# xiezheng-cs/PyTorch_Distributed_Template

Hardware: AMD Instinct MI355X
Metric: images/sec (node) ResNet-18 DDP bs=1200/GPU at 1/2/4/8 MI355X (higher is better)
Workload: dtype bf16; 1 GPU; model=resnet18, global_batch=1200, parallelism=dp1, per_gpu_batch=1200, sync_bn=False, engine=native-hip, comm=none, grad_compress=none

## Files before the change

csrc/bindings.cpp:

```cpp
#include <torch/extension.h>
#include <ATen/hip/HIPContext.h>
#include <c10/hip/HIPCachingAllocator.h>
#include <c10/hip/HIPGuard.h>

#include <cstdio>
#include <algorithm>
#include <map>
#include <memory>
#include <mutex>
#include <optional>
#include <vector>
#include <stdexcept>
#include <string>

#include "common.h"
#include "dtypes.h"
#include "kernels/bn.h"
#include "kernels/bnact.h"
#include "kernels/conv1x1.h"
#include "kernels/conv_fwd.h"
#include "kernels/conv_l1.h"
#include "kernels/conv_wgrad.h"
#include "kernels/dwconv.h"
#include "kernels/fp32.h"
// ... 130 lines not shown
    TORCH_CHECK(Pm > 0 && Qm > 0 && f[6] + C * f[2] * f[3] * K + (nslice - 1) * w_slice_stride <= w_numel, op,
                ": bad phase");
    a.pooff_h[i] = (int)f[0]; a.pooff_w[i] = (int)f[1]; a.pT[i] = (int)f[2]; a.pU[i] = (int)f[3];
    a.pioff_h[i] = (int)f[4]; a.pioff_w[i] = (int)f[5]; a.pwoff[i] = f[6];
    a.pPm[i] = (int)Pm; a.pQm[i] = (int)Qm;
    maxM = std::max(maxM, N * Pm * Qm);
  }
  TORCH_CHECK(maxM < (int64_t(1) << 31), op, ": N*Pm*Qm must be < 2^31 (32-bit pixel indexing)");
  a.M = maxM;
}

void conv_fwd(const Tensor& x, const Tensor& w, Tensor& y, const OptT& res, const OptT& stats, int64_t N, int64_t H,
              int64_t W, int64_t C, int64_t Kout, int64_t T, int64_t U, int64_t Pm, int64_t Qm, int64_t ist_h,
              int64_t ist_w, int64_t ioff_h, int64_t ioff_w, int64_t tstep_h, int64_t tstep_w, int64_t OH, int64_t OW,
              int64_t ost_h, int64_t ost_w, int64_t ooff_h, int64_t ooff_w, int64_t bm, int64_t bn, int64_t bk,
              int64_t cs) {
  const int dt = dt16(x, "x");
  if (cs <= 0) cs = C;
  TORCH_CHECK(dt16(w, "w") == dt && dt16(y, "y") == dt, "conv_fwd: mixed dtypes");
  TORCH_CHECK(x.numel() == N * H * W * cs, "conv_fwd: x has ", x.numel(), " elements, geometry needs ", N * H * W * cs);
  TORCH_CHECK(x.numel() < (int64_t(1) << 30) && w.numel() < (int64_t(1) << 30),
              "conv_fwd: operands exceed 2 GiB (32-bit buffer offsets)");
  int pair_skip = 0;
  if (cs != C) {
    const int rows = C == 64 ? 2 : 1;
    TORCH_CHECK(cs == 4 && (C == 32 || (C == 64 && bk == 64 && U == 1)) && tstep_w >= 0 && U >= 1 && ioff_h >= 0 &&
                    ioff_w >= 0 && (Pm - 1) * ist_h + ioff_h + (T - 1) * tstep_h + rows - 1 < H &&
                    ((Qm - 1) * ist_w + ioff_w + (U - 1) * tstep_w) * cs + 32 <= W * cs,
                "conv_fwd: window-mode geometry leaves the padded image");
    if (C == 64) pair_skip = (int)(W * cs - 32);
  }
  TORCH_CHECK(w.numel() == Kout * T * U * C, "conv_fwd: w size mismatch");
// ... 8 lines not shown
  if (res.has_value()) {
    TORCH_CHECK(res->numel() == y.numel(), "conv_fwd: residual size mismatch");
    a.res = p16(*res, "res");
  }
  const int64_t M = N * Pm * Qm;
  if (stats.has_value()) {
    TORCH_CHECK(stats->numel() >= pdt::kStatSlots * Kout * 2, "conv_fwd: stats buffer too small");
    a.stats = pd(*stats, "stats");
  }
  a.N = N; a.H = H; a.W = W; a.C = C; a.Kout = Kout; a.T = T; a.U = U; a.Pm = Pm; a.Qm = Qm; a.cs = cs;
  a.pair_skip = pair_skip;
  a.ist_h = ist_h; a.ist_w = ist_w; a.ioff_h = ioff_h; a.ioff_w = ioff_w; a.tstep_h = tstep_h; a.tstep_w = tstep_w;
  a.OH = OH; a.OW = OW; a.ost_h = ost_h; a.ost_w = ost_w; a.ooff_h = ooff_h; a.ooff_w = ooff_w;
  TORCH_CHECK(M < (int64_t(1) << 31), "conv_fwd: N*Pm*Qm must be < 2^31 (32-bit pixel indexing)");
  a.M = M;
  pdt::conv_fwd_launch(a, dt, (int)bm, (int)bn, (int)bk, cur_stream());
  launched("conv_fwd_launch");
}

bool conv_fwd_pre_supported(int64_t N, int64_t H, int64_t W) {
  pdt::ConvFwdArgs a{};
  set_fwd_geom(a, N, H, W, 64, 64, 3, 3, H, W, 1, 1);
  a.cs = 64;
  int flip = 0;
  return pdt::conv_l1_eligible(a, &flip);
}

void conv_fwd_pre(const Tensor& z, const Tensor& w, Tensor& y, const Tensor& stats, const Tensor& pre_coef, int64_t N,
                  int64_t H, int64_t W) {
  const int dt = dt16(z, "z");
// ... 49 lines not shown
                              int64_t Q, int64_t res_phase) {
  if (!(bnb == 2 || bnb == 3) || res_phase >= 0 || stride != 1 || phases.size() != 1 || H != P || W != Q) return 0;
  const auto& f = phases[0];
  if (f.size() < 6 || f[0] != 0 || f[1] != 0 || f[2] != 1 || f[3] != 1 || f[4] != 0 || f[5] != 0) return 0;
  const bool x_ok = pdt::conv1x1x_bnb_supported((int)K, (int)C);
  if ((K == 64 || (K == 128 && bnb == 2)) && C == 256 && pdt::conv1x1_c64_supported(64, C) &&
      !(pdt::conv1x1x_prefer_l1() && x_ok))
    return 1;
  return x_ok ? 2 : 0;
}

void conv_dgrad_impl(const Tensor& dy, const Tensor& wt, Tensor& dx, const OptT& res, int64_t N, int64_t P,
                     int64_t Q, int64_t K, int64_t C, int64_t H, int64_t W, int64_t stride,
                     const std::vector<std::vector<int64_t>>& phases, int64_t bm, int64_t bn, int64_t bk, int64_t bnb,
                     const OptT& bn_y1, const OptT& bn_coef1, const OptT& bn_y2, const OptT& bn_coef2,
                     const OptT& bn_mask, const OptT& bn_slots, int64_t res_phase) {
  const int dt = dt16(dy, "dy");
  TORCH_CHECK(dt16(wt, "wt") == dt && dt16(dx, "dx") == dt, "conv_dgrad: mixed dtypes");
  TORCH_CHECK(dy.numel() == N * P * Q * K && dx.numel() == N * H * W * C, "conv_dgrad: size mismatch");
  TORCH_CHECK(dy.numel() < (int64_t(1) << 30) && wt.numel() < (int64_t(1) << 30),
              "conv_dgrad: operands exceed 2 GiB (32-bit buffer offsets)");
  TORCH_CHECK(K % bk == 0 && C % bn == 0, "conv_dgrad: K % bk / C % bn must be 0");
  pdt::ConvFwdArgs a{};
  a.x = p16(dy, "dy");
  a.w = p16(wt, "wt");
  a.y = p16(dx, "dx");
  set_dgrad_geom("conv_dgrad", a, N, P, Q, K, C, H, W, stride, phases, wt.numel(), 1, 0);
  a.cs = K;
  TORCH_CHECK(res_phase < (int64_t)phases.size() && (res_phase < 0 || res.has_value()), "conv_dgrad: bad res_phase");
  if (res.has_value()) {
    if (res_phase >= 0) {
      const int64_t Pm = a.pPm[res_phase], Qm = a.pQm[res_phase];
// ... 31 lines not shown
  const int64_t pk = dgrad_persistent_kind(K, C, bnb, stride, phases, H, W, P, Q, res_phase);
  if (pk == 1) {
    pdt::conv1x1_c64_bnb_launch(a.x, a.w + a.pwoff[0], a.y, a.res, a.bn_y1, a.bn_coef1, bnb == 3 ? a.bn_y2 : nullptr,
                                bnb == 3 ? a.bn_coef2 : nullptr, a.bn_mask, a.stats, N * P * Q, (int)K, dt,
                                cur_stream());
    launched("conv1x1_c64_bnb");
    return;
  }
  if (pk == 2) {
    pdt::conv1x1x_bnb_launch(a.x, a.w + a.pwoff[0], a.y, a.res, a.bn_y1, a.bn_coef1, bnb == 3 ? a.bn_y2 : nullptr,
                             bnb == 3 ? a.bn_coef2 : nullptr, a.bn_mask, a.stats, N * P * Q, (int)K, (int)C, dt,
                             cur_stream());
    launched("conv1x1x_bnb");
    return;
  }
  pdt::conv_fwd_launch(a, dt, (int)bm, (int)bn, (int)bk, cur_stream());
  launched("conv_fwd_launch");
}

void conv_dgrad(const Tensor& dy, const Tensor& wt, Tensor& dx, const OptT& res, int64_t N, int64_t P, int64_t Q,
                int64_t K, int64_t C, int64_t H, int64_t W, int64_t stride, const std::vector<std::vector<int64_t>>& phases,
                int64_t bm, int64_t bn, int64_t bk) {
  conv_dgrad_impl(dy, wt, dx, res, N, P, Q, K, C, H, W, stride, phases, bm, bn, bk, 0, {}, {}, {}, {}, {}, {}, -1);
}

bool conv1x1_c64_supported(int64_t C, int64_t Kout) { return pdt::conv1x1_c64_supported((int)C, (int)Kout); }

void conv1x1_c64(const Tensor& x, const Tensor& w, Tensor& y, const OptT& stats, int64_t M, const OptT& pre) {
  const int dt = dt16(x, "x");
  TORCH_CHECK(dt16(w, "w") == dt && dt16(y, "y") == dt, "conv1x1_c64: mixed dtypes");
  TORCH_CHECK(x.numel() >= M * 64 && w.numel() == 256 * 64 && y.numel() >= M * 256, "conv1x1_c64: size mismatch");
  TORCH_CHECK(M * 256 < (int64_t(1) << 31), "conv1x1_c64: M*256 must be < 2^31 (32-bit buffer offsets)");
  double* st = nullptr;
  if (stats.has_value()) {
    TORCH_CHECK(stats->numel() >= pdt::kStatSlots * 256 * 2, "conv1x1_c64: stats buffer too small");
    st = pd(*stats, "stats");
  }
  const float* pc = nullptr;
// ... 1066 lines not shown
  pdt_store::register_store(m);
  pdt_dp::register_dp(m);
  m.doc() = "gfx950 (MI355X) HIP kernels of pytorch_distributed_template_amd";
  m.def("dispatch_counts", []() {
    std::map<std::string, long long> out;
    auto& r = pdt::counters();
    std::lock_guard<std::mutex> lk(r.mu);
    for (auto& e : r.entries) out[e.first] = __atomic_load_n(e.second.get(), __ATOMIC_RELAXED);
    return out;
  });
  m.def("reset_dispatch_counts", []() {
    auto& r = pdt::counters();
    std::lock_guard<std::mutex> lk(r.mu);
    for (auto& e : r.entries) __atomic_store_n(e.second.get(), 0LL, __ATOMIC_RELAXED);
  });
  m.def("conv_fwd", &conv_fwd);
  m.def("conv_m_tiles", &conv_m_tiles);
  m.def("conv_dgrad", &conv_dgrad);
  m.def("conv_dgrad_bn", &conv_dgrad_impl);
  m.def("conv_wgrad_plan", &conv_wgrad_plan);
  m.def("conv1x1_c64_supported", &conv1x1_c64_supported);
  m.def("conv1x1_c64", &conv1x1_c64, py::arg("x"), py::arg("w"), py::arg("y"), py::arg("stats"), py::arg("M"),
        py::arg("pre") = py::none());
  m.def("conv1x1_c64_mode", [](int64_t set) { return (int64_t)pdt::conv1x1_c64_mode((int)set); });
  m.def("conv_wgrad", &conv_wgrad, py::arg("x"), py::arg("dy"), py::arg("ws"), py::arg("N"), py::arg("H"), py::arg("W"),
        py::arg("C"), py::arg("Kout"), py::arg("T"), py::arg("U"), py::arg("Pm"), py::arg("Qm"), py::arg("stride_h"),
        py::arg("stride_w"), py::arg("pad_h"), py::arg("pad_w"), py::arg("dil_h"), py::arg("dil_w"), py::arg("ldw"),
        py::arg("splits"), py::arg("pix_per_split"), py::arg("cs"), py::arg("win"), py::arg("pre") = py::none());
  m.def("conv_wgrad_stem_fused", &conv_wgrad_stem_fused);
  m.def("gconv_fwd", &gconv_fwd);
  m.def("gconv_dgrad", &gconv_dgrad, py::arg("dy"), py::arg("wt"), py::arg("dx"), py::arg("N"), py::arg("P"),
        py::arg("Q"), py::arg("width"), py::arg("H"), py::arg("W"), py::arg("stride"), py::arg("phases"), py::arg("j"),
        py::arg("bm"), py::arg("bn"), py::arg("bn_y1") = py::none(), py::arg("bn_coef1") = py::none(),
        py::arg("bn_slots") = py::none());
// ... 109 lines not shown
```

csrc/kernels/conv_fwd.h:

```cpp
#pragma once
#include <hip/hip_runtime.h>
#include <stdint.h>

#include "conv_geom.h"

namespace pdt {

constexpr int kStatSlots = 64;

void stat_rows_reduce_launch(const float* rows, int R, int CK, double* slots, hipStream_t s, int slots_ld = 0);


struct ConvFwdArgs : ConvGeom {
  const uint16_t* x;
  const uint16_t* w;
  uint16_t* y;
  const uint16_t* res;
  double* stats;
  int bnb;
  const uint16_t* bn_y1;
  const float* bn_coef1;
  const uint16_t* bn_y2;
  const float* bn_coef2;
  const uint8_t* bn_mask;
  int pair_skip;
  int res_phase = -1;
  int stage_out = 0;
  const float* pre_coef = nullptr;
  int ldy = 0, coef_ld = 0, stats_ld = 0;
  int nslice = 0;
  int64_t slice_wstride = 0;
  int srows_coff = 0;
};

void conv_fwd_launch(const ConvFwdArgs& a, int dtype, int bm, int bn, int bk, hipStream_t s);
int conv_fwd_m_tiles(int64_t M, int bm);

}
```

csrc/kernels/conv_fwd.hip:

```cpp
#include <cstdlib>

#include "../common.h"
#include "conv_fwd.h"
#include "conv_l1.h"

namespace pdt {

typedef __attribute__((address_space(3))) void lds_void;
typedef __attribute__((address_space(1))) void glb_void;

template <int CHUNKS>
PDT_DEVICE int swz(int row) { return (row >> 1) & (CHUNKS - 1); }

template <int DT, int EPI, int RES, int FN, int FM, int WN, int WM, int BN, int WAVES_M, int NW_, int SMEM = 0,
          bool PERM = false>
PDT_DEVICE void conv_epilogue(const ConvFwdArgs& a, f32x4_t (&acc)[FN][FM], int64_t m0, int n0, int tile_m, int wn,
                              int wm, int tid, int lane, char* smem) {
  using E = E16<DT>;
  const int fr = lane & 15, fq = lane >> 4;
  const int PQ = a.Pm * a.Qm;
  const FastDiv fd_pq{a.pq_mul, a.pq_shift}, fd_q{a.q_mul, a.q_shift};
  constexpr int KS = EPI == 0 ? 0 : (EPI == 4 ? 3 : 2);
  float sacc[FN][4][KS > 0 ? KS : 1];
#pragma unroll
  for (int i = 0; i < FN; ++i)
#pragma unroll
    for (int r = 0; r < 4; ++r)
#pragma unroll
      for (int k = 0; k < (KS > 0 ? KS : 1); ++k) sacc[i][r][k] = 0.f;

  constexpr int RED_BYTES = WAVES_M * BN * 3 * 4;
  float* cf = (float*)(smem + RED_BYTES);
// ... 26 lines not shown
                     : (8 * PER_J <= BUDGET && FM % 8 == 0) ? 8
                     : (4 * PER_J <= BUDGET && FM % 4 == 0) ? 4
                     : (2 * PER_J <= BUDGET && FM % 2 == 0) ? 2 : 1;
  static_assert(FM % JC == 0, "epilogue chunking");
  constexpr int BM_T = WAVES_M * WM;
  constexpr int SPITCH = BN * 2 + 16;
  constexpr int STG_OFF = 16384;
  constexpr bool FULL = SMEM >= STG_OFF + BM_T * SPITCH;
  constexpr bool PERGRP = !FULL && WAVES_M > 1 && EPI != 2 && SMEM >= STG_OFF + WM * SPITCH;
  constexpr bool CAN_STAGE = FULL || PERGRP;
  static_assert(!CAN_STAGE || RED_BYTES + 6 * BN * 4 <= STG_OFF, "epilogue LDS regions overlap");
  const bool stage = CAN_STAGE && a.stage_out;
  char* stg = smem + STG_OFF;
  const int srow0 = FULL ? wm * WM : 0;
  constexpr bool RC = RES == 2;
  const bool res_on = !RC || (int)blockIdx.y == a.res_phase;
  auto copy_rows = [&](int g) {
    constexpr int CPR = BN / 8;
    constexpr int SROWS = FULL ? BM_T : WM;
    for (int q = tid; q < SROWS * CPR; q += NW_ * 64) {
      const int row = q / CPR, ch = q - row * CPR;
      const int64_t m = m0 + (FULL ? 0 : g * WM) + row;
      if (m < a.M) {
        const int mm = (int)m;
        const int nimg = (int)fdiv((uint32_t)mm, fd_pq);
        const int rem = mm - nimg * PQ;
        const int i_ = (int)fdiv((uint32_t)rem, fd_q), j_ = rem - i_ * a.Qm;
        const int oh = i_ * a.ost_h + a.ooff_h, ow = j_ * a.ost_w + a.ooff_w;
        const int64_t ob = (((int64_t)nimg * a.OH + oh) * a.OW + ow) * LDY + n0 + ch * 8;
        *(uint4*)(a.y + ob) = *(const uint4*)(stg + row * SPITCH + ch * 16);
      }
// ... 184 lines not shown
        for (int r = 0; r < 4; ++r) {
          const int nl = wn * WN + chan(i, r);
#pragma unroll
          for (int k = 0; k < KS; ++k) red[(wm * BN + nl) * KS + k] = sacc[i][r][k];
        }
    }
    __syncthreads();
    if (tid < BN) {
      float t[KS];
#pragma unroll
      for (int k = 0; k < KS; ++k) t[k] = 0.f;
#pragma unroll
      for (int w = 0; w < WAVES_M; ++w)
#pragma unroll
        for (int k = 0; k < KS; ++k) t[k] += red[(w * BN + tid) * KS + k];
      const int64_t row = (a.nphase > 0 ? (int64_t)blockIdx.y * a.srows_pp : 0) + tile_m;
      const int64_t sld = a.nslice > 1 ? (int64_t)a.nslice * a.Kout : a.Kout;
      float* dst = a.srows + (row * sld + a.srows_coff + n0 + tid) * KO;
      if constexpr (EPI == 4)
        *(float4*)dst = make_float4(t[0], t[1], t[0], t[2]);
      else
        *(float2*)dst = make_float2(t[0], t[1]);
    }
  }
}

template <int EPI, int BN_>
PDT_DEVICE void zero_stat_row(const ConvFwdArgs& a, int nthreads) {
  if constexpr (EPI != 0) {
    constexpr int KO = EPI == 4 ? 4 : 2;
    const int tm = (int)blockIdx.x / a.n_tiles, tn = (int)blockIdx.x - tm * a.n_tiles;
    const int64_t sld = a.nslice > 1 ? (int64_t)a.nslice * a.Kout : a.Kout;
    float* dst = a.srows + (((int64_t)blockIdx.y * a.srows_pp + tm) * sld + a.srows_coff) * KO + (int64_t)tn * BN_ * KO;
    for (int i = threadIdx.x; i < BN_ * KO; i += nthreads) dst[i] = 0.f;
  }
}

template <int DT, int BM, int BN, int BK, int WAVES_N, int EPI, int RES, int STAGES, int NW>
__global__ __launch_bounds__(NW * 64, (STAGES * (BN + BM) * BK * 2 <= 81920 || NW == 8) ? 2 : 1)
void conv_fwd_kernel(ConvFwdArgs args) {
  ConvFwdArgs a = args;
  const uint16_t* wbase = args.w;
  if (args.nslice > 1) {
    const int sl = blockIdx.z;
    a.x += (int64_t)sl * a.Kout;
    a.y += (int64_t)sl * a.Kout;
    wbase += (int64_t)sl * args.slice_wstride;
    a.w = wbase;
    if (a.bn_y1 != nullptr) a.bn_y1 += (int64_t)sl * a.Kout;
    if (a.bn_coef1 != nullptr) a.bn_coef1 += sl * a.Kout;
    a.srows_coff = sl * a.Kout;
  }
  if (args.nphase > 0 && !select_phase(a, args, wbase, blockIdx.y)) {
    zero_stat_row<EPI, BN>(a, NW * 64);
    return;
  }
  using E = E16<DT>;
  typedef typename E::vec8 vec8;
  constexpr int WAVES_M = NW / WAVES_N;
  constexpr int WN = BN / WAVES_N;
  constexpr int WM = BM / WAVES_M;
  constexpr int FN = WN / 16, FM = WM / 16;
  constexpr int ROWB = BK * 2;
  constexpr int CHUNKS = ROWB / 16;
  constexpr int RPI = 1024 / ROWB;
  constexpr int A_INSTR = BN / RPI / NW;
  constexpr int B_INSTR = BM / RPI / NW;
  constexpr int A_BYTES = BN * ROWB;
  constexpr int STAGE = (BN + BM) * ROWB;
// ... 147 lines not shown
        const int ahead = min(S - 2, ksteps - 1 - ks);
        wait_ahead(ahead);
        __builtin_amdgcn_s_barrier();
        if (ks + S - 1 < ksteps) stage_load(buf == 0 ? S - 1 : buf - 1);
        __builtin_amdgcn_s_setprio(1);
        compute_stage(smem + buf * STAGE);
        __builtin_amdgcn_s_setprio(0);
        buf = buf == S - 1 ? 0 : buf + 1;
      }
      asm volatile("s_waitcnt lgkmcnt(0)" ::: "memory");
      __builtin_amdgcn_s_barrier();
    }
  }

  conv_epilogue<DT, EPI, RES, FN, FM, WN, WM, BN, WAVES_M, NW, STAGES * STAGE, PERM>(a, acc, m0, n0, tile_m, wn, wm, tid,
                                                                             lane, smem);
}

template <int N>
PDT_DEVICE void vm_wait() {
  static_assert(N >= 0 && N < 64, "vmcnt range");
  __builtin_amdgcn_s_waitcnt((N & 0xF) | ((N >> 4) << 14) | (0x7 << 4) | (0xF << 8));
}

template <int DT, int BM, int BN, int EPI, int RES, bool PP_STAGE = (EPI != 2)>
__global__ __launch_bounds__(512) void conv_pp_kernel(ConvFwdArgs args) {
  ConvFwdArgs a = args;
  if (args.nphase > 0 && !select_phase(a, args, args.w, blockIdx.y)) {
    zero_stat_row<EPI, BN>(a, 512);
    return;
  }
  using E = E16<DT>;
  typedef typename E::vec8 vec8;
  constexpr int NW = 8, WN = 64, WM = 128;
  constexpr int WAVES_N = BN / WN, WAVES_M = NW / WAVES_N;
  static_assert(WAVES_N * WAVES_M == NW && WAVES_M * WM == BM, "pp tile geometry");
  constexpr int FN = 4, FM = 8;
  constexpr int ROWB = 128;
  constexpr int XH = (BM / 2) * ROWB;
  constexpr int WH = (BN / 2) * ROWB;
  constexpr int NX = XH / 1024 / NW;
  constexpr int NWI = WH / 1024 / NW;
  static_assert(NX * 1024 * NW == XH && NWI * 1024 * NW == WH, "pp DMA split");
  constexpr int BUF = 2 * XH + 2 * WH;
  constexpr int OX0 = 0, OX1 = XH, OW0 = 2 * XH, OW1 = 2 * XH + WH;
  __shared__ __attribute__((aligned(1024))) char smem[2 * BUF];

  const int tid = threadIdx.x;
  const int lane = tid & 63;
  const int wave = __builtin_amdgcn_readfirstlane(tid >> 6);
  const int grp = wave >> 2;
  const int wn = wave % WAVES_N, wm = wave / WAVES_N;

  const int nwg = a.m_tiles * a.n_tiles;
  const int bid = xcd_remap(blockIdx.x, nwg);
  const int tile_m = bid / a.n_tiles, tile_n = bid % a.n_tiles;
  const int64_t m0 = (int64_t)tile_m * BM;
  const int n0 = tile_n * BN;

  const int PQ = a.Pm * a.Qm;
  const FastDiv fd_pq{a.pq_mul, a.pq_shift}, fd_q{a.q_mul, a.q_shift};
  const int TU = a.T * a.U;
  const int csteps = a.C >> 6;
  const int ksteps = TU * csteps;

  const __amdgpu_buffer_rsrc_t rx = make_rsrc(a.x, (uint32_t)a.N * a.H * a.W * a.cs * 2u);
  const __amdgpu_buffer_rsrc_t rw = make_rsrc(a.w, (uint32_t)a.Kout * TU * a.C * 2u);

  const int lrow = lane >> 3, pchunk = lane & 7;
  int xhw[2][NX], xoff[2][NX];
#pragma unroll
  for (int h = 0; h < 2; ++h)
#pragma unroll
    for (int j = 0; j < NX; ++j) {
      const int hr = (wave * NX + j) * 8 + lrow;
      const int64_t m = m0 + (hr >> 6) * 128 + h * 64 + (hr & 63);
      const int bch = pchunk ^ ((hr >> 1) & 7);
      if (m < a.M) {
        const int nimg = (int)fdiv((uint32_t)m, fd_pq);
        const int rem = (int)m - nimg * PQ;
        const int i = (int)fdiv((uint32_t)rem, fd_q), jj = rem - i * a.Qm;
        const int ih = i * a.ist_h + a.ioff_h, iw = jj * a.ist_w + a.ioff_w;
        xhw[h][j] = (ih << 16) | (iw & 0xffff);
        xoff[h][j] = (((nimg * a.H + ih) * a.W + iw) * a.cs + bch * 8) * 2;
      } else {
        xhw[h][j] = (int)0xC0000000;
        xoff[h][j] = 0;
      }
    }
  uint32_t woff[2][NWI];
#pragma unroll
  for (int h = 0; h < 2; ++h)
#pragma unroll
    for (int j = 0; j < NWI; ++j) {
      const int hr = (wave * NWI + j) * 8 + lrow;
      const int lr = hr & 31;
      const int n = n0 + (hr >> 5) * 64 + h * 32 + ((lr & 15) >> 2) * 8 + (lr >> 4) * 4 + (lr & 3);
      woff[h][j] = (uint32_t)((n * TU * a.C + (pchunk ^ ((hr >> 1) & 7)) * 8) * 2);
    }

  int cur_t = 0, cur_u = 0, cur_c = 0;
  uint32_t s_adelta = 0;
  int s_dh = 0, s_dw = 0, s_bdelta = 0;
  auto advance = [&]() {
    s_adelta = (uint32_t)((cur_t * a.U + cur_u) * a.C + cur_c) * 2u;
    s_dh = cur_t * a.tstep_h;
    s_dw = cur_u * a.tstep_w;
    s_bdelta = ((s_dh * a.W + s_dw) * a.cs + cur_c) * 2;
    cur_c += 64;
    if (cur_c == a.C) {
      cur_c = 0;
      if (++cur_u == a.U) { cur_u = 0; ++cur_t; }
    }
  };
  auto dma_x = [&](char* buf, int h) {
#pragma unroll
    for (int j = 0; j < NX; ++j) {
      const int ih = (xhw[h][j] >> 16) + s_dh, iw = (int)(short)(xhw[h][j] & 0xffff) + s_dw;
      const bool ok = (unsigned)ih < (unsigned)a.H && (unsigned)iw < (unsigned)a.W;
      buf_lds16(rx, buf + (h ? OX1 : OX0) + (wave * NX + j) * 1024, ok ? (uint32_t)(xoff[h][j] + s_bdelta) : kOOB);
    }
  };
  auto dma_w = [&](char* buf, int h) {
#pragma unroll
    for (int j = 0; j < NWI; ++j)
      buf_lds16(rw, buf + (h ? OW1 : OW0) + (wave * NWI + j) * 1024, woff[h][j] + s_adelta);
  };

  f32x4_t acc[FN][FM];
#pragma unroll
  for (int i = 0; i < FN; ++i)
#pragma unroll
    for (int j = 0; j < FM; ++j) acc[i][j] = f32x4_t{0.f, 0.f, 0.f, 0.f};

  const int fr = lane & 15, fq = lane >> 4;
  const int xrow0 = wm * 64 + fr, wrow0 = wn * 32 + fr;
  const int sw = (fr >> 1) & 7;
  vec8 xs[4][2], w0r[2][2], w1r[2][2];
  auto read_x = [&](const char* base) {
#pragma unroll
    for (int f = 0; f < 4; ++f)
#pragma unroll
      for (int kk = 0; kk < 2; ++kk)
        xs[f][kk] = *(const vec8*)(base + (xrow0 + f * 16) * ROWB + (((kk * 4 + fq) ^ sw) << 4));
  };
  auto read_w = [&](vec8 (&wr)[2][2], const char* base) {
#pragma unroll
    for (int f = 0; f < 2; ++f)
#pragma unroll
      for (int kk = 0; kk < 2; ++kk)
        wr[f][kk] = *(const vec8*)(base + (wrow0 + f * 16) * ROWB + (((kk * 4 + fq) ^ sw) << 4));
  };
// ... 6 lines not shown
        for (int f = 0; f < 4; ++f)
          acc[wh * 2 + f2][xh * 4 + f] = E::mfma16x16x32(wr[f2][kk], xs[f][kk], acc[wh * 2 + f2][xh * 4 + f]);
  };
  auto compute = [&](const vec8 (&wr)[2][2], int xh, int wh) {
    __builtin_amdgcn_sched_barrier(0);
    __builtin_amdgcn_s_barrier();
    __builtin_amdgcn_sched_barrier(0);
    __builtin_amdgcn_s_setprio(1);
    mma(wr, xh, wh);
    __builtin_amdgcn_s_setprio(0);
    __builtin_amdgcn_sched_barrier(0);
    __builtin_amdgcn_s_barrier();
    __builtin_amdgcn_sched_barrier(0);
  };

  if (ksteps > 0) {
    advance();
    dma_x(smem, 0);
    dma_w(smem, 0);
    dma_w(smem, 1);
    dma_x(smem, 1);
    vm_wait<NWI + NX>();
    __builtin_amdgcn_sched_barrier(0);
    __builtin_amdgcn_s_barrier();
    if (grp == 1) __builtin_amdgcn_s_barrier();
    for (int ks = 0; ks < ksteps; ++ks) {
      const char* cb = smem + (ks & 1) * BUF;
      char* nb = smem + ((ks + 1) & 1) * BUF;
      const bool more = ks + 1 < ksteps;
      if (more) advance();
      if (more) { dma_x(nb, 0); vm_wait<2 * NX>(); } else { vm_wait<NX>(); }
      read_x(cb + OX0);
      read_w(w0r, cb + OW0);
      compute(w0r, 0, 0);
      if (more) { dma_w(nb, 0); vm_wait<NX + NWI>(); } else { vm_wait<0>(); }
      read_w(w1r, cb + OW1);
      compute(w1r, 0, 1);
      if (more) dma_w(nb, 1);
      read_x(cb + OX1);
      compute(w1r, 1, 1);
      if (more) { dma_x(nb, 1); vm_wait<NWI + NX>(); }
      compute(w0r, 1, 0);
    }
    if (grp == 0) __builtin_amdgcn_s_barrier();
    asm volatile("s_waitcnt vmcnt(0) lgkmcnt(0)" ::: "memory");
    __builtin_amdgcn_s_barrier();
  }

  conv_epilogue<DT, EPI, RES, FN, FM, WN, WM, BN, WAVES_M, NW, PP_STAGE ? 2 * BUF : 0, true>(a, acc, m0, n0, tile_m, wn,
                                                                                        wm, tid, lane, smem);
}

template <int DT, int BM, int BN>
static void launch_pp(const ConvFwdArgs& args, int gx, hipStream_t s) {
  ConvFwdArgs a = args;
  a.stage_out = 0;
  if (a.nslice > 1)
    pdt_hip_fail("conv_pp: slice-batched (grouped) launches run on the generic kernel", hipErrorInvalidValue, __FILE__,
                 __LINE__);
  dim3 grid(gx, a.nphase > 0 ? a.nphase : 1), block(512);
  const int rs = a.res == nullptr ? 0 : (a.res_phase >= 0 && a.nphase > 0 ? 2 : 1);
  const int epi = a.bnb ? a.bnb + 1 : (a.stats != nullptr ? 1 : 0);
#define PDT_K(E_, R_) hipLaunchKernelGGL((conv_pp_kernel<DT, BM, BN, E_, R_>), grid, block, 0, s, a)
  if (epi == 0) {
    if (rs == 1) PDT_K(0, 1); else if (rs == 2) PDT_K(0, 2); else PDT_K(0, 0);
  } else if (epi == 1 && rs != 2) {
    if (rs) PDT_K(1, 1); else PDT_K(1, 0);
  } else if (epi == 2 && !rs) {
    PDT_K(2, 0);
  } else if (epi == 3 && rs) {
    if (rs == 2) PDT_K(3, 2); else PDT_K(3, 1);
  } else if (epi == 4 && rs) {
    if (rs == 2) PDT_K(4, 2); else PDT_K(4, 1);
  } else {
    pdt_hip_fail("conv_pp: unsupported epilogue variant", hipErrorInvalidValue, __FILE__, __LINE__);
// ... 146 lines not shown
```

pytorch_distributed_template_amd/ops/conv.py:

```python
from __future__ import annotations

from typing import List, Optional, Tuple

import torch

from . import native


_PP_MIN_K = 128


_WIDE128_MIN_TILES = 1024


def conv_tile(cout: int, kdim: int = 0, m: int = 0) -> Tuple[int, int]:
    if cout % 256 == 0 and kdim >= _PP_MIN_K and kdim % 64 == 0:
        return 256, 256
    if cout % 128 == 0:
        if m and (m + 255) // 256 * (cout // 128) >= _WIDE128_MIN_TILES:
            return 256, 128
        return 128, 128
    return 256, 64


# ... 11 lines not shown
def dgrad_weight_index(cout: int, cin: int, R: int, S: int, rs: List[int], ss: List[int]) -> torch.Tensor:
    if not rs or not ss:
        return torch.empty(0, dtype=torch.long)
    c = torch.arange(cin).view(-1, 1, 1, 1)
    t = torch.tensor(rs).view(1, -1, 1, 1)
    u = torch.tensor(ss).view(1, 1, -1, 1)
    k = torch.arange(cout).view(1, 1, 1, -1)
    return (((k * R + t) * S + u) * cin + c).reshape(-1)


def out_hw(H: int, W: int, R: int, S: int, stride: int, pad: int) -> Tuple[int, int]:
    return (H + 2 * pad - R) // stride + 1, (W + 2 * pad - S) // stride + 1


def conv_fwd(x: torch.Tensor, w: torch.Tensor, stride: int = 1, pad: int = 0, stats: bool = False,
             residual: Optional[torch.Tensor] = None, tile: Optional[Tuple[int, int, int]] = None):
    N, H, W, C = x.shape
    K, R, S, C2 = w.shape
    assert C == C2
    P, Q = out_hw(H, W, R, S, stride, pad)
    y = torch.empty(N, P, Q, K, dtype=x.dtype, device=x.device)
    bm, bn = conv_tile(K, C * R * S, N * P * Q)
    bk = 64 if C % 64 == 0 else 32
    if tile is not None:
        bm, bn, bk = tile
    sp = None
    if stats:
        sp = torch.empty(native.C.stat_slots() * K * 2, dtype=torch.float64, device=x.device)
    native.C.conv_fwd(x, w, y, residual, sp, N, H, W, C, K, R, S, P, Q, stride, stride, -pad, -pad, 1, 1,
                      P, Q, 1, 1, 0, 0, bm, bn, bk, 0)
    if not stats:
        return y
    sums = torch.empty(2 * K, dtype=torch.float64, device=x.device)
    native.C.bn_slot_sum(sp, K, 2, sums)
    return y, (sums[:K], sums[K:])


def pack_relu_mask(out: torch.Tensor) -> torch.Tensor:
    bits = (out.reshape(-1, 8) > 0).to(torch.int32)
    w = (1 << torch.arange(8, device=out.device, dtype=torch.int32))
    return (bits * w).sum(1).to(torch.uint8)


def conv_dgrad(dy: torch.Tensor, w: torch.Tensor, H: int, W: int, stride: int = 1, pad: int = 0,
               residual: Optional[torch.Tensor] = None, bnb: Optional[tuple] = None,
               tile: Optional[Tuple[int, int, int]] = None, res_phase: int = -1) -> torch.Tensor:
    N, P, Q, K = dy.shape
    K2, R, S, C = w.shape
    assert K == K2
    dx = torch.empty(N, H, W, C, dtype=dy.dtype, device=dy.device)
    bm, bn = conv_tile(C, K * R * S, N * H * W)
    bk = 64 if K % 64 == 0 else 32
    if tile is not None:
        bm, bn, bk = tile
    wflat = w.reshape(-1)
    pieces, phases, off = [], [], 0
    for ph, pw, rs, ss, ioff_h, ioff_w in dgrad_phases(R, S, stride, pad):
        if H - ph <= 0 or W - pw <= 0:
            continue
        idx = dgrad_weight_index(K, C, R, S, rs, ss).to(w.device)
        if idx.numel():
            pieces.append(wflat[idx])
        phases.append([ph, pw, len(rs), len(ss), ioff_h, ioff_w, off])
        off += idx.numel()
    wt = torch.cat(pieces).contiguous() if pieces else torch.zeros(1, dtype=w.dtype, device=w.device)
    if bnb is None and res_phase < 0:
        native.C.conv_dgrad(dy, wt, dx, residual, N, P, Q, K, C, H, W, stride, phases, bm, bn, bk)
    else:
        native.C.conv_dgrad_bn(dy, wt, dx, residual, N, P, Q, K, C, H, W, stride, phases, bm, bn, bk,
                               *(bnb or (0, None, None, None, None, None, None)), res_phase)
    return dx


def conv_wgrad(x: torch.Tensor, dy: torch.Tensor, R: int, S: int, stride: int = 1, pad: int = 0,
               target_blocks: int = 2048) -> torch.Tensor:
    N, H, W, C = x.shape
    _, P, Q, K = dy.shape
    splits, pps, _ = native.C.conv_wgrad_plan(K, R, S, C, N * P * Q, target_blocks, False)
    ldw = R * S * C
    ws = torch.empty(splits * K * ldw, dtype=torch.float32, device=x.device)
    native.C.conv_wgrad(x, dy, ws, N, H, W, C, K, R, S, P, Q, stride, stride, pad, pad, 1, 1, ldw, splits, pps, 0,
                        False)
    out = torch.empty(K * ldw, dtype=torch.float32, device=x.device)
    native.C.wgrad_reduce(ws, splits, K, ldw, ldw, K * ldw, out, ldw, 1.0, False)
    return out.view(K, R, S, C)
# ... 1 lines not shown
```

Baseline: 62610 images/s.

## Make conv_pp kernel persistent with next-tile prefetch overlapping the epilogue

```diff
diff --git a/csrc/bindings.cpp b/csrc/bindings.cpp
--- a/csrc/bindings.cpp
+++ b/csrc/bindings.cpp
@@ -168,8 +168,9 @@
               int64_t W, int64_t C, int64_t Kout, int64_t T, int64_t U, int64_t Pm, int64_t Qm, int64_t ist_h,
               int64_t ist_w, int64_t ioff_h, int64_t ioff_w, int64_t tstep_h, int64_t tstep_w, int64_t OH, int64_t OW,
               int64_t ost_h, int64_t ost_w, int64_t ooff_h, int64_t ooff_w, int64_t bm, int64_t bn, int64_t bk,
-              int64_t cs) {
+              int64_t cs, int64_t max_wg) {
   const int dt = dt16(x, "x");
+  TORCH_CHECK(max_wg >= 0 && max_wg < (int64_t(1) << 30), "conv_fwd: bad max_wg");
   if (cs <= 0) cs = C;
   TORCH_CHECK(dt16(w, "w") == dt && dt16(y, "y") == dt, "conv_fwd: mixed dtypes");
   TORCH_CHECK(x.numel() == N * H * W * cs, "conv_fwd: x has ", x.numel(), " elements, geometry needs ", N * H * W * cs);
@@ -208,6 +209,7 @@
   a.OH = OH; a.OW = OW; a.ost_h = ost_h; a.ost_w = ost_w; a.ooff_h = ooff_h; a.ooff_w = ooff_w;
   TORCH_CHECK(M < (int64_t(1) << 31), "conv_fwd: N*Pm*Qm must be < 2^31 (32-bit pixel indexing)");
   a.M = M;
+  a.max_wg = (int)max_wg;
   pdt::conv_fwd_launch(a, dt, (int)bm, (int)bn, (int)bk, cur_stream());
   launched("conv_fwd_launch");
 }
@@ -287,8 +289,9 @@
                      int64_t Q, int64_t K, int64_t C, int64_t H, int64_t W, int64_t stride,
                      const std::vector<std::vector<int64_t>>& phases, int64_t bm, int64_t bn, int64_t bk, int64_t bnb,
                      const OptT& bn_y1, const OptT& bn_coef1, const OptT& bn_y2, const OptT& bn_coef2,
-                     const OptT& bn_mask, const OptT& bn_slots, int64_t res_phase) {
+                     const OptT& bn_mask, const OptT& bn_slots, int64_t res_phase, int64_t max_wg) {
   const int dt = dt16(dy, "dy");
+  TORCH_CHECK(max_wg >= 0 && max_wg < (int64_t(1) << 30), "conv_dgrad: bad max_wg");
   TORCH_CHECK(dt16(wt, "wt") == dt && dt16(dx, "dx") == dt, "conv_dgrad: mixed dtypes");
   TORCH_CHECK(dy.numel() == N * P * Q * K && dx.numel() == N * H * W * C, "conv_dgrad: size mismatch");
   TORCH_CHECK(dy.numel() < (int64_t(1) << 30) && wt.numel() < (int64_t(1) << 30),
@@ -350,6 +353,7 @@
     launched("conv1x1x_bnb");
     return;
   }
+  a.max_wg = (int)max_wg;
   pdt::conv_fwd_launch(a, dt, (int)bm, (int)bn, (int)bk, cur_stream());
   launched("conv_fwd_launch");
 }
@@ -357,7 +361,7 @@
 void conv_dgrad(const Tensor& dy, const Tensor& wt, Tensor& dx, const OptT& res, int64_t N, int64_t P, int64_t Q,
                 int64_t K, int64_t C, int64_t H, int64_t W, int64_t stride, const std::vector<std::vector<int64_t>>& phases,
                 int64_t bm, int64_t bn, int64_t bk) {
-  conv_dgrad_impl(dy, wt, dx, res, N, P, Q, K, C, H, W, stride, phases, bm, bn, bk, 0, {}, {}, {}, {}, {}, {}, -1);
+  conv_dgrad_impl(dy, wt, dx, res, N, P, Q, K, C, H, W, stride, phases, bm, bn, bk, 0, {}, {}, {}, {}, {}, {}, -1, 0);
 }
 
 bool conv1x1_c64_supported(int64_t C, int64_t Kout) { return pdt::conv1x1_c64_supported((int)C, (int)Kout); }
@@ -1454,10 +1458,18 @@
     std::lock_guard<std::mutex> lk(r.mu);
     for (auto& e : r.entries) __atomic_store_n(e.second.get(), 0LL, __ATOMIC_RELAXED);
   });
-  m.def("conv_fwd", &conv_fwd);
+  m.def("conv_fwd", &conv_fwd, py::arg("x"), py::arg("w"), py::arg("y"), py::arg("res"), py::arg("stats"), py::arg("N"),
+        py::arg("H"), py::arg("W"), py::arg("C"), py::arg("Kout"), py::arg("T"), py::arg("U"), py::arg("Pm"), py::arg("Qm"),
+        py::arg("ist_h"), py::arg("ist_w"), py::arg("ioff_h"), py::arg("ioff_w"), py::arg("tstep_h"), py::arg("tstep_w"),
+        py::arg("OH"), py::arg("OW"), py::arg("ost_h"), py::arg("ost_w"), py::arg("ooff_h"), py::arg("ooff_w"),
+        py::arg("bm"), py::arg("bn"), py::arg("bk"), py::arg("cs"), py::arg("max_wg") = 0);
   m.def("conv_m_tiles", &conv_m_tiles);
   m.def("conv_dgrad", &conv_dgrad);
-  m.def("conv_dgrad_bn", &conv_dgrad_impl);
+  m.def("conv_dgrad_bn", &conv_dgrad_impl, py::arg("dy"), py::arg("wt"), py::arg("dx"), py::arg("res"), py::arg("N"),
+        py::arg("P"), py::arg("Q"), py::arg("K"), py::arg("C"), py::arg("H"), py::arg("W"), py::arg("stride"),
+        py::arg("phases"), py::arg("bm"), py::arg("bn"), py::arg("bk"), py::arg("bnb"), py::arg("bn_y1"),
+        py::arg("bn_coef1"), py::arg("bn_y2"), py::arg("bn_coef2"), py::arg("bn_mask"), py::arg("bn_slots"),
+        py::arg("res_phase"), py::arg("max_wg") = 0);
   m.def("conv_wgrad_plan", &conv_wgrad_plan);
   m.def("conv1x1_c64_supported", &conv1x1_c64_supported);
   m.def("conv1x1_c64", &conv1x1_c64, py::arg("x"), py::arg("w"), py::arg("y"), py::arg("stats"), py::arg("M"),
diff --git a/csrc/kernels/conv_fwd.h b/csrc/kernels/conv_fwd.h
--- a/csrc/kernels/conv_fwd.h
+++ b/csrc/kernels/conv_fwd.h
@@ -31,6 +31,7 @@
   int nslice = 0;
   int64_t slice_wstride = 0;
   int srows_coff = 0;
+  int max_wg = 0;
 };
 
 void conv_fwd_launch(const ConvFwdArgs& a, int dtype, int bm, int bn, int bk, hipStream_t s);
diff --git a/csrc/kernels/conv_fwd.hip b/csrc/kernels/conv_fwd.hip
--- a/csrc/kernels/conv_fwd.hip
+++ b/csrc/kernels/conv_fwd.hip
@@ -15,7 +15,7 @@
 template <int DT, int EPI, int RES, int FN, int FM, int WN, int WM, int BN, int WAVES_M, int NW_, int SMEM = 0,
           bool PERM = false>
 PDT_DEVICE void conv_epilogue(const ConvFwdArgs& a, f32x4_t (&acc)[FN][FM], int64_t m0, int n0, int tile_m, int wn,
-                              int wm, int tid, int lane, char* smem) {
+                              int wm, int tid, int lane, char* smem, int ph) {
   using E = E16<DT>;
   const int fr = lane & 15, fq = lane >> 4;
   const int PQ = a.Pm * a.Qm;
@@ -72,7 +72,7 @@
   char* stg = smem + STG_OFF;
   const int srow0 = FULL ? wm * WM : 0;
   constexpr bool RC = RES == 2;
-  const bool res_on = !RC || (int)blockIdx.y == a.res_phase;
+  const bool res_on = !RC || ph == a.res_phase;
   auto copy_rows = [&](int g) {
     constexpr int CPR = BN / 8;
     constexpr int SROWS = FULL ? BM_T : WM;
@@ -287,7 +287,7 @@
       for (int w = 0; w < WAVES_M; ++w)
 #pragma unroll
         for (int k = 0; k < KS; ++k) t[k] += red[(w * BN + tid) * KS + k];
-      const int64_t row = (a.nphase > 0 ? (int64_t)blockIdx.y * a.srows_pp : 0) + tile_m;
+      const int64_t row = (a.nphase > 0 ? (int64_t)ph * a.srows_pp : 0) + tile_m;
       const int64_t sld = a.nslice > 1 ? (int64_t)a.nslice * a.Kout : a.Kout;
       float* dst = a.srows + (row * sld + a.srows_coff + n0 + tid) * KO;
       if constexpr (EPI == 4)
@@ -299,12 +299,12 @@
 }
 
 template <int EPI, int BN_>
-PDT_DEVICE void zero_stat_row(const ConvFwdArgs& a, int nthreads) {
+PDT_DEVICE void zero_stat_row(const ConvFwdArgs& a, int nthreads, int slot, int ph) {
   if constexpr (EPI != 0) {
     constexpr int KO = EPI == 4 ? 4 : 2;
-    const int tm = (int)blockIdx.x / a.n_tiles, tn = (int)blockIdx.x - tm * a.n_tiles;
+    const int tm = slot / a.n_tiles, tn = slot - tm * a.n_tiles;
     const int64_t sld = a.nslice > 1 ? (int64_t)a.nslice * a.Kout : a.Kout;
-    float* dst = a.srows + (((int64_t)blockIdx.y * a.srows_pp + tm) * sld + a.srows_coff) * KO + (int64_t)tn * BN_ * KO;
+    float* dst = a.srows + (((int64_t)ph * a.srows_pp + tm) * sld + a.srows_coff) * KO + (int64_t)tn * BN_ * KO;
     for (int i = threadIdx.x; i < BN_ * KO; i += nthreads) dst[i] = 0.f;
   }
 }
@@ -325,7 +325,7 @@
     a.srows_coff = sl * a.Kout;
   }
   if (args.nphase > 0 && !select_phase(a, args, wbase, blockIdx.y)) {
-    zero_stat_row<EPI, BN>(a, NW * 64);
+    zero_stat_row<EPI, BN>(a, NW * 64, (int)blockIdx.x, (int)blockIdx.y);
     return;
   }
   using E = E16<DT>;
@@ -503,7 +503,7 @@
   }
 
   conv_epilogue<DT, EPI, RES, FN, FM, WN, WM, BN, WAVES_M, NW, STAGES * STAGE, PERM>(a, acc, m0, n0, tile_m, wn, wm, tid,
-                                                                             lane, smem);
+                                                                             lane, smem, (int)blockIdx.y);
 }
 
 template <int N>
@@ -512,13 +512,8 @@
   __builtin_amdgcn_s_waitcnt((N & 0xF) | ((N >> 4) << 14) | (0x7 << 4) | (0xF << 8));
 }
 
-template <int DT, int BM, int BN, int EPI, int RES, bool PP_STAGE = (EPI != 2)>
+template <int DT, int BM, int BN, int EPI, int RES>
 __global__ __launch_bounds__(512) void conv_pp_kernel(ConvFwdArgs args) {
-  ConvFwdArgs a = args;
-  if (args.nphase > 0 && !select_phase(a, args, args.w, blockIdx.y)) {
-    zero_stat_row<EPI, BN>(a, 512);
-    return;
-  }
   using E = E16<DT>;
   typedef typename E::vec8 vec8;
   constexpr int NW = 8, WN = 64, WM = 128;
@@ -541,72 +536,86 @@
   const int grp = wave >> 2;
   const int wn = wave % WAVES_N, wm = wave / WAVES_N;
 
-  const int nwg = a.m_tiles * a.n_tiles;
-  const int bid = xcd_remap(blockIdx.x, nwg);
-  const int tile_m = bid / a.n_tiles, tile_n = bid % a.n_tiles;
-  const int64_t m0 = (int64_t)tile_m * BM;
-  const int n0 = tile_n * BN;
-
-  const int PQ = a.Pm * a.Qm;
-  const FastDiv fd_pq{a.pq_mul, a.pq_shift}, fd_q{a.q_mul, a.q_shift};
-  const int TU = a.T * a.U;
-  const int csteps = a.C >> 6;
-  const int ksteps = TU * csteps;
-
-  const __amdgpu_buffer_rsrc_t rx = make_rsrc(a.x, (uint32_t)a.N * a.H * a.W * a.cs * 2u);
-  const __amdgpu_buffer_rsrc_t rw = make_rsrc(a.w, (uint32_t)a.Kout * TU * a.C * 2u);
-
-  const int lrow = lane >> 3, pchunk = lane & 7;
+  const int G = (int)gridDim.x;
+  const int slots = args.srows_pp * args.n_tiles;
+  const int total = (args.nphase > 0 ? args.nphase : 1) * slots;
+  auto decode = [&](ConvFwdArgs& g, int item, int& ph, int& slot) {
+    ph = 0;
+    slot = item;
+    if (args.nphase > 0) {
+      ph = (item >= slots) + (item >= 2 * slots) + (item >= 3 * slots);
+      slot = item - ph * slots;
+      select_phase(g, args, args.w, ph);
+    }
+    return slot < g.m_tiles * g.n_tiles;
+  };
+  auto ksteps_of = [](const ConvFwdArgs& g) { return g.T * g.U * (g.C >> 6); };
+
+  const __amdgpu_buffer_rsrc_t rx = make_rsrc(args.x, (uint32_t)args.N * args.H * args.W * args.cs * 2u);
+  __amdgpu_buffer_rsrc_t rw = make_rsrc(args.w, 0u);
+
+  int lrow = 0, pchunk = 0;
   int xhw[2][NX], xoff[2][NX];
-#pragma unroll
-  for (int h = 0; h < 2; ++h)
-#pragma unroll
-    for (int j = 0; j < NX; ++j) {
-      const int hr = (wave * NX + j) * 8 + lrow;
-      const int64_t m = m0 + (hr >> 6) * 128 + h * 64 + (hr & 63);
-      const int bch = pchunk ^ ((hr >> 1) & 7);
-      if (m < a.M) {
-        const int nimg = (int)fdiv((uint32_t)m, fd_pq);
-        const int rem = (int)m - nimg * PQ;
-        const int i = (int)fdiv((uint32_t)rem, fd_q), jj = rem - i * a.Qm;
-        const int ih = i * a.ist_h + a.ioff_h, iw = jj * a.ist_w + a.ioff_w;
-        xhw[h][j] = (ih << 16) | (iw & 0xffff);
-        xoff[h][j] = (((nimg * a.H + ih) * a.W + iw) * a.cs + bch * 8) * 2;
-      } else {
-        xhw[h][j] = (int)0xC0000000;
-        xoff[h][j] = 0;
-      }
-    }
   uint32_t woff[2][NWI];
-#pragma unroll
-  for (int h = 0; h < 2; ++h)
-#pragma unroll
-    for (int j = 0; j < NWI; ++j) {
-      const int hr = (wave * NWI + j) * 8 + lrow;
-      const int lr = hr & 31;
-      const int n = n0 + (hr >> 5) * 64 + h * 32 + ((lr & 15) >> 2) * 8 + (lr >> 4) * 4 + (lr & 3);
-      woff[h][j] = (uint32_t)((n * TU * a.C + (pchunk ^ ((hr >> 1) & 7)) * 8) * 2);
-    }
-
-  int cur_t = 0, cur_u = 0, cur_c = 0;
+  int cur_t = 0, cur_u = 0, cur_c = 0, ld_U = 1;
   uint32_t s_adelta = 0;
   int s_dh = 0, s_dw = 0, s_bdelta = 0;
+  auto setup = [&](const ConvFwdArgs& g, int slot) {
+    const int bid = xcd_remap(slot, g.m_tiles * g.n_tiles);
+    const int tm = bid / g.n_tiles;
+    const int64_t m0 = (int64_t)tm * BM;
+    const int n0 = (bid - tm * g.n_tiles) * BN;
+    const int PQ = g.Pm * g.Qm;
+    const FastDiv fd_pq{g.pq_mul, g.pq_shift}, fd_q{g.q_mul, g.q_shift};
+    const int TU = g.T * g.U;
+    rw = make_rsrc(g.w, (uint32_t)g.Kout * TU * g.C * 2u);
+#pragma unroll
+    for (int h = 0; h < 2; ++h)
+#pragma unroll
+      for (int j = 0; j < NX; ++j) {
+        const int hr = (wave * NX + j) * 8 + lrow;
+        const int64_t m = m0 + (hr >> 6) * 128 + h * 64 + (hr & 63);
+        const int bch = pchunk ^ ((hr >> 1) & 7);
+        if (m < g.M) {
+          const int nimg = (int)fdiv((uint32_t)m, fd_pq);
+          const int rem = (int)m - nimg * PQ;
+          const int i = (int)fdiv((uint32_t)rem, fd_q), jj = rem - i * g.Qm;
+          const int ih = i * g.ist_h + g.ioff_h, iw = jj * g.ist_w + g.ioff_w;
+          xhw[h][j] = (ih << 16) | (iw & 0xffff);
+          xoff[h][j] = (((nimg * g.H + ih) * g.W + iw) * g.cs + bch * 8) * 2;
+        } else {
+          xhw[h][j] = (int)0xC0000000;
+          xoff[h][j] = 0;
+        }
+      }
+#pragma unroll
+    for (int h = 0; h < 2; ++h)
+#pragma unroll
+      for (int j = 0; j < NWI; ++j) {
+        const int hr = (wave * NWI + j) * 8 + lrow;
+        const int lr = hr & 31;
+        const int n = n0 + (hr >> 5) * 64 + h * 32 + ((lr & 15) >> 2) * 8 + (lr >> 4) * 4 + (lr & 3);
+        woff[h][j] = (uint32_t)((n * TU * g.C + (pchunk ^ ((hr >> 1) & 7)) * 8) * 2);
+      }
+    cur_t = 0; cur_u = 0; cur_c = 0;
+    ld_U = g.U;
+  };
   auto advance = [&]() {
-    s_adelta = (uint32_t)((cur_t * a.U + cur_u) * a.C + cur_c) * 2u;
-    s_dh = cur_t * a.tstep_h;
-    s_dw = cur_u * a.tstep_w;
-    s_bdelta = ((s_dh * a.W + s_dw) * a.cs + cur_c) * 2;
+    s_adelta = (uint32_t)((cur_t * ld_U + cur_u) * args.C + cur_c) * 2u;
+    s_dh = cur_t * args.tstep_h;
+    s_dw = cur_u * args.tstep_w;
+    s_bdelta = ((s_dh * args.W + s_dw) * args.cs + cur_c) * 2;
     cur_c += 64;
-    if (cur_c == a.C) {
+    if (cur_c == args.C) {
       cur_c = 0;
-      if (++cur_u == a.U) { cur_u = 0; ++cur_t; }
+      if (++cur_u == ld_U) { cur_u = 0; ++cur_t; }
     }
   };
   auto dma_x = [&](char* buf, int h) {
 #pragma unroll
     for (int j = 0; j < NX; ++j) {
       const int ih = (xhw[h][j] >> 16) + s_dh, iw = (int)(short)(xhw[h][j] & 0xffff) + s_dw;
-      const bool ok = (unsigned)ih < (unsigned)a.H && (unsigned)iw < (unsigned)a.W;
+      const bool ok = (unsigned)ih < (unsigned)args.H && (unsigned)iw < (unsigned)args.W;
       buf_lds16(rx, buf + (h ? OX1 : OX0) + (wave * NX + j) * 1024, ok ? (uint32_t)(xoff[h][j] + s_bdelta) : kOOB);
     }
   };
@@ -615,16 +624,17 @@
     for (int j = 0; j < NWI; ++j)
       buf_lds16(rw, buf + (h ? OW1 : OW0) + (wave * NWI + j) * 1024, woff[h][j] + s_adelta);
   };
+  auto dma_step0 = [&](char* buf) {
+    advance();
+    dma_x(buf, 0);
+    dma_w(buf, 0);
+    dma_w(buf, 1);
+    dma_x(buf, 1);
+  };
 
   f32x4_t acc[FN][FM];
-#pragma unroll
-  for (int i = 0; i < FN; ++i)
-#pragma unroll
-    for (int j = 0; j < FM; ++j) acc[i][j] = f32x4_t{0.f, 0.f, 0.f, 0.f};
-
-  const int fr = lane & 15, fq = lane >> 4;
-  const int xrow0 = wm * 64 + fr, wrow0 = wn * 32 + fr;
-  const int sw = (fr >> 1) & 7;
+
+  int fq = 0, xrow0 = 0, wrow0 = 0, sw = 0;
   vec8 xs[4][2], w0r[2][2], w1r[2][2];
   auto read_x = [&](const char* base) {
 #pragma unroll
@@ -661,19 +671,50 @@
     __builtin_amdgcn_sched_barrier(0);
   };
 
+  int par = 0;
+  bool have = false;
+  for (int item = (int)blockIdx.x; item < total; item += G) {
+    int item_o = item;
+    asm volatile("" : "+s"(item_o));
+    ConvFwdArgs a = args;
+    int ph = 0, slot = 0;
+    if (!decode(a, item_o, ph, slot)) {
+      zero_stat_row<EPI, BN>(a, 512, slot, ph);
+      continue;
+    }
+    const int bid = xcd_remap(slot, a.m_tiles * a.n_tiles);
+    const int tile_m = bid / a.n_tiles, tile_n = bid - tile_m * a.n_tiles;
+    const int64_t m0 = (int64_t)tile_m * BM;
+    const int n0 = tile_n * BN;
+    const int ksteps = ksteps_of(a);
+    {
+      int lane_o = lane;
+      asm volatile("" : "+v"(lane_o));
+      const int fr = lane_o & 15;
+      lrow = lane_o >> 3; pchunk = lane_o & 7;
+      fq = lane_o >> 4; xrow0 = wm * 64 + fr; wrow0 = wn * 32 + fr;
+      sw = (fr >> 1) & 7;
+    }
+#pragma unroll
+    for (int i = 0; i < FN; ++i)
+#pragma unroll
+      for (int j = 0; j < FM; ++j) acc[i][j] = f32x4_t{0.f, 0.f, 0.f, 0.f};
+
   if (ksteps > 0) {
-    advance();
-    dma_x(smem, 0);
-    dma_w(smem, 0);
-    dma_w(smem, 1);
-    dma_x(smem, 1);
-    vm_wait<NWI + NX>();
+    setup(a, slot);
+    if (!have) {
+      dma_step0(smem + par * BUF);
+      vm_wait<NWI + NX>();
+    } else {
+      advance();
+      vm_wait<0>();
+    }
     __builtin_amdgcn_sched_barrier(0);
     __builtin_amdgcn_s_barrier();
     if (grp == 1) __builtin_amdgcn_s_barrier();
     for (int ks = 0; ks < ksteps; ++ks) {
-      const char* cb = smem + (ks & 1) * BUF;
-      char* nb = smem + ((ks + 1) & 1) * BUF;
+      const char* cb = smem + ((par + ks) & 1) * BUF;
+      char* nb = smem + ((par + ks + 1) & 1) * BUF;
       const bool more = ks + 1 < ksteps;
       if (more) advance();
       if (more) { dma_x(nb, 0); vm_wait<2 * NX>(); } else { vm_wait<NX>(); }
@@ -693,9 +734,22 @@
     asm volatile("s_waitcnt vmcnt(0) lgkmcnt(0)" ::: "memory");
     __builtin_amdgcn_s_barrier();
   }
-
-  conv_epilogue<DT, EPI, RES, FN, FM, WN, WM, BN, WAVES_M, NW, PP_STAGE ? 2 * BUF : 0, true>(a, acc, m0, n0, tile_m, wn,
-                                                                                        wm, tid, lane, smem);
+    const int sb = ksteps > 0 ? (par + ksteps - 1) & 1 : par ^ 1;
+    have = false;
+    if (item + G < total) {
+      ConvFwdArgs an = args;
+      int nph = 0, nslot = 0;
+      if (decode(an, item + G, nph, nslot) && ksteps_of(an) > 0) {
+        setup(an, nslot);
+        dma_step0(smem + (sb ^ 1) * BUF);
+        have = true;
+      }
+    }
+    par = sb ^ 1;
+    conv_epilogue<DT, EPI, RES, FN, FM, WN, WM, BN, WAVES_M, NW, 0, true>(a, acc, m0, n0, tile_m, wn, wm, tid, lane,
+                                                                         smem + sb * BUF, ph);
+    vm_wait<0>();
+  }
 }
 
 template <int DT, int BM, int BN>
@@ -705,7 +759,24 @@
   if (a.nslice > 1)
     pdt_hip_fail("conv_pp: slice-batched (grouped) launches run on the generic kernel", hipErrorInvalidValue, __FILE__,
                  __LINE__);
-  dim3 grid(gx, a.nphase > 0 ? a.nphase : 1), block(512);
+  static const int persist = [] {
+    const char* e = getenv("PDT_PP_PERSIST");
+    return e && e[0] ? atoi(e) : 3;
+  }();
+  static const int cus = [] {
+    int dev = 0, n = 0;
+    if (hipGetDevice(&dev) != hipSuccess || hipDeviceGetAttribute(&n, hipDeviceAttributeMultiprocessorCount, dev) != hipSuccess)
+      n = 256;
+    return n > 0 ? n : 256;
+  }();
+  const int total = gx * (a.nphase > 0 ? a.nphase : 1);
+  int G = total;
+  if (a.max_wg > 0)
+    G = a.max_wg;
+  else if (persist & (a.nphase > 0 ? 2 : 1))
+    G = cus;
+  if (G > total) G = total;
+  dim3 grid(G), block(512);
   const int rs = a.res == nullptr ? 0 : (a.res_phase >= 0 && a.nphase > 0 ? 2 : 1);
   const int epi = a.bnb ? a.bnb + 1 : (a.stats != nullptr ? 1 : 0);
 #define PDT_K(E_, R_) hipLaunchKernelGGL((conv_pp_kernel<DT, BM, BN, E_, R_>), grid, block, 0, s, a)
diff --git a/pytorch_distributed_template_amd/ops/conv.py b/pytorch_distributed_template_amd/ops/conv.py
--- a/pytorch_distributed_template_amd/ops/conv.py
+++ b/pytorch_distributed_template_amd/ops/conv.py
@@ -49,7 +49,8 @@
 
 
 def conv_fwd(x: torch.Tensor, w: torch.Tensor, stride: int = 1, pad: int = 0, stats: bool = False,
-             residual: Optional[torch.Tensor] = None, tile: Optional[Tuple[int, int, int]] = None):
+             residual: Optional[torch.Tensor] = None, tile: Optional[Tuple[int, int, int]] = None,
+             max_wg: int = 0):
     N, H, W, C = x.shape
     K, R, S, C2 = w.shape
     assert C == C2
@@ -63,7 +64,7 @@
     if stats:
         sp = torch.empty(native.C.stat_slots() * K * 2, dtype=torch.float64, device=x.device)
     native.C.conv_fwd(x, w, y, residual, sp, N, H, W, C, K, R, S, P, Q, stride, stride, -pad, -pad, 1, 1,
-                      P, Q, 1, 1, 0, 0, bm, bn, bk, 0)
+                      P, Q, 1, 1, 0, 0, bm, bn, bk, 0, max_wg)
     if not stats:
         return y
     sums = torch.empty(2 * K, dtype=torch.float64, device=x.device)
@@ -79,7 +80,7 @@
 
 def conv_dgrad(dy: torch.Tensor, w: torch.Tensor, H: int, W: int, stride: int = 1, pad: int = 0,
                residual: Optional[torch.Tensor] = None, bnb: Optional[tuple] = None,
-               tile: Optional[Tuple[int, int, int]] = None, res_phase: int = -1) -> torch.Tensor:
+               tile: Optional[Tuple[int, int, int]] = None, res_phase: int = -1, max_wg: int = 0) -> torch.Tensor:
     N, P, Q, K = dy.shape
     K2, R, S, C = w.shape
     assert K == K2
@@ -99,11 +100,11 @@
         phases.append([ph, pw, len(rs), len(ss), ioff_h, ioff_w, off])
         off += idx.numel()
     wt = torch.cat(pieces).contiguous() if pieces else torch.zeros(1, dtype=w.dtype, device=w.device)
-    if bnb is None and res_phase < 0:
+    if bnb is None and res_phase < 0 and max_wg == 0:
         native.C.conv_dgrad(dy, wt, dx, residual, N, P, Q, K, C, H, W, stride, phases, bm, bn, bk)
     else:
         native.C.conv_dgrad_bn(dy, wt, dx, residual, N, P, Q, K, C, H, W, stride, phases, bm, bn, bk,
-                               *(bnb or (0, None, None, None, None, None, None)), res_phase)
+                               *(bnb or (0, None, None, None, None, None, None)), res_phase, max_wg)
     return dx
 
 
```

Measured after the change: 63340 images/s (median of 6 runs). +1.2%, better.
